# chen-bowen/instacart_next_order_recommendation

Measured on AMD Instinct MI355X. Metric: recommend_qps_top20_49k7_catalog, higher is better.
Workload: dtype f16x3 (f32 operands split into 2 f16 planes, 3 f16 MFMAs per product, f32 accumulate; fp32-level accuracy)

## Files before the change

### instacart_next_order_recommendation_amd/csrc/encoder.hip

```cpp
#include <stdlib.h>

#include <mutex>
#include <type_traits>
#include <vector>

#include "common.h"
#include "gemm_x3.h"
#include "wt_gemm.h"
#include "encoder_x3.h"

namespace icrec {

__device__ __forceinline__ int find_seq(const int32_t* __restrict__ cu, int n_seqs, int t) {
    int lo = 0, hi = n_seqs;
    while (hi - lo > 1) {
        int mid = (lo + hi) >> 1;
        if (cu[mid] <= t) lo = mid; else hi = mid;
    }
    return lo;
}

template <int H, bool SPLIT>
__device__ __forceinline__ void ln_row(float (&v)[H / 64], const float* __restrict__ g, const float* __restrict__ b,
                                       float eps, float* __restrict__ out, _Float16* __restrict__ oh,
// ... 263 lines not shown
#pragma unroll
    for (int j = 0; j < 8; ++j) {
        const _Float16 a = (_Float16)x[j];
        hi[j] = a;
        lo[j] = (_Float16)((x[j] - (float)a) * LO_SCALE);
    }
}

__device__ __forceinline__ half4 lds_read_tr(const _Float16* p) {
    typedef __fp16 fp16x4 __attribute__((__vector_size__(4 * sizeof(__fp16))));
    return __builtin_bit_cast(half4, __builtin_amdgcn_ds_read_tr16_b64_v4f16(
                                         (__attribute__((address_space(3))) fp16x4*)(reinterpret_cast<uintptr_t>(p))));
}

template <int NKT, int WAVES, bool SPLIT>
__global__ __launch_bounds__(WAVES * 64, (NKT >= 6 ? 4 : NKT == 4 ? 3 : 1)) void attention_x3_kernel(const float* __restrict__ qkv,
                                                                  const int32_t* __restrict__ cu, int heads, int H,
                                                                  float scale_log2e, float* __restrict__ ctx,
                                                                  _Float16* __restrict__ ch, _Float16* __restrict__ cl,
                                                                  const int32_t* __restrict__ order, int nlo) {
    constexpr bool RECOMP = NKT >= 6;
    __shared__ __attribute__((aligned(16))) _Float16 Kbuf[2 * NKT * 32 * 32];
    _Float16* const Kh = Kbuf;
    _Float16* const Kl = Kbuf + NKT * 32 * 32;
    __shared__ __attribute__((aligned(16))) _Float16 Vh[NKT * 32 * 32];
    __shared__ __attribute__((aligned(16))) _Float16 Vl[NKT * 32 * 32];
    __shared__ float Ls[WAVES * 32];
    constexpr bool OB = SPLIT;
    static_assert(!OB || WAVES * 2 * 32 * 32 <= 2 * NKT * 32 * 32, "the output tiles reuse the K planes");
    _Float16* const Ob = Kbuf;

    const int tid = threadIdx.x, lane = tid & 63, wave = tid >> 6;
    const int sidx = blockIdx.x / heads, hd = blockIdx.x % heads;
    const int s = order != nullptr ? order[sidx] : sidx;
    const int t0 = cu[s], L = cu[s + 1] - t0;
    const int nkt = (L + 31) >> 5;
    if (nkt > NKT || nkt <= nlo) return;
    const int qb0 = blockIdx.y * WAVES;
    if (qb0 >= nkt) return;
    const int ld = 3 * H;

    const int r = lane & 31, h = lane >> 5;
    const int qb = qb0 + wave;
    ICREC_STAMP(0, 0);
    half8 qh[2], ql[2];
    {
        int qr = qb * 32 + r;
        qr = qr < L ? qr : L - 1;
        const float* qp = qkv + (size_t)(t0 + qr) * ld + hd * DH;
#pragma unroll
        for (int ks = 0; ks < 2; ++ks) {
            const f32x4 a = *reinterpret_cast<const f32x4*>(qp + 16 * ks + 8 * h);
            const f32x4 b = *reinterpret_cast<const f32x4*>(qp + 16 * ks + 8 * h + 4);
            half4 ah, al, bh, bl;
            split_act4(a, ah, al);
            split_act4(b, bh, bl);
            qh[ks] = half8{ah[0], ah[1], ah[2], ah[3], bh[0], bh[1], bh[2], bh[3]};
            ql[ks] = half8{al[0], al[1], al[2], al[3], bl[0], bl[1], bl[2], bl[3]};
        }
    }
    ICREC_STAMP(0, 6);
    constexpr int STG = NKT * 32 * 8 / (WAVES * 64);
    static_assert(NKT * 32 * 8 % (WAVES * 64) == 0, "staging: whole rounds");
    f32x4 kreg[STG], vreg[STG];
#pragma unroll
    for (int it = 0; it < STG; ++it) {
        const int id = tid + it * WAVES * 64;
        const int key = id >> 3, c = id & 7;
        const int rr = key < L ? key : L - 1;
        const float* src = qkv + (size_t)(t0 + rr) * ld + hd * DH + c * 4;
        kreg[it] = *reinterpret_cast<const f32x4*>(src + H);
        vreg[it] = *reinterpret_cast<const f32x4*>(src + 2 * H);
    }
#ifdef ICREC_STAMPS
    asm volatile("s_waitcnt vmcnt(0)" ::: "memory");
    ICREC_STAMP(0, 7);
#endif
#pragma unroll
    for (int it = 0; it < STG; ++it) {
        const int id = tid + it * WAVES * 64;
        if (id < nkt * 32 * 8) {
            const int key = id >> 3, c = id & 7;
            half4 khi, klo, vhi, vlo;
            split_act4(kreg[it], khi, klo);
            split_act4(vreg[it], vhi, vlo);
            *reinterpret_cast<half4*>(Vh + key * 32 + c * 4) = vhi;
            *reinterpret_cast<half4*>(Vl + key * 32 + c * 4) = vlo;
            const int off = key * 32 + ((((c >> 1) ^ ((key >> 2) & 3)) << 3) | ((c & 1) << 2));
            *reinterpret_cast<half4*>(Kh + off) = khi;
            *reinterpret_cast<half4*>(Kl + off) = klo;
        }
    }
    ICREC_STAMP(0, 1);
    __syncthreads();
    ICREC_STAMP(0, 2);
    const bool active = qb < nkt;
    if (!RECOMP && !OB && !active) return;

    auto score_tile = [&](int kt, bool hi_only = false) {
        f32x16 t;
#pragma unroll
        for (int e = 0; e < 16; ++e) t[e] = 0.0f;
        const int key = kt * 32 + r;
#pragma unroll
        for (int ks = 0; ks < 2; ++ks) {
            const int off = key * 32 + (((2 * ks + h) ^ ((key >> 2) & 3)) << 3);
            const half8 kh = *reinterpret_cast<const half8*>(Kh + off);
// ... 300 lines not shown
    const long long v = strtoll(s, &end, 10);
    if (end == s) return fallback;
    return (int)(v < 0 ? 0 : v > hi ? hi : v);
}

template <bool GELU>
static void launch_linear(const float* A, int M, int K, const float* W, int N, const float* bias, float* out,
                          hipStream_t st) {
    const int mt = (M + GemmBig::BM - 1) / GemmBig::BM, nt = (N + GemmBig::BN - 1) / GemmBig::BN;
    hipLaunchKernelGGL((linear_kernel<GemmBig, GELU>), dim3(mt * nt), dim3(GemmBig::THREADS), 0, st, A, M, K, W, N,
                       bias, out, nt);
}

template <int EPI>
static void launch_wt_linear(const _Float16* Xh, const _Float16* Xl, int T, int K, const _Float16* Wp, int N,
                             const float* bias, float* out, _Float16* oh, _Float16* ol, hipStream_t st, int small_m) {
    if (T <= small_m) {
        if constexpr (EPI == 0 || EPI == 2) {
            if (N % 64 == 0 && K % 128 == 0) {
                const int nbn = N / 64;
                if (K % 256 == 0 && K >= 1024)
                    hipLaunchKernelGGL((wt_linear_half_kernel<EPI, 8>), dim3(((T + 31) / 32) * nbn), dim3(256), 0, st, Xh, Xl, T, K, Wp,
                                       N, bias, out, (const _Float16*)oh, (const _Float16*)ol, nbn);
                else if (K % 384 == 0)
                    hipLaunchKernelGGL((wt_linear_half_kernel<EPI, 6>), dim3(((T + 31) / 32) * nbn), dim3(256), 0, st, Xh, Xl, T, K, Wp,
                                       N, bias, out, (const _Float16*)oh, (const _Float16*)ol, nbn);
                else
                hipLaunchKernelGGL((wt_linear_half_kernel<EPI>), dim3(((T + 31) / 32) * nbn), dim3(256), 0, st, Xh, Xl, T, K, Wp, N,
                                   bias, out, (const _Float16*)oh, (const _Float16*)ol, nbn);
                return;
            }
        }
        const int nbn = N / 128;
        hipLaunchKernelGGL((wt_linear_kernel<1, 1, 4, EPI>), dim3(((T + 31) / 32) * nbn), dim3(256), 0, st, Xh, Xl, T, K,
                           Wp, N, bias, out, oh, ol, nbn);
    } else {
        const int nbn = N / 384;
        hipLaunchKernelGGL((wt_linear_kernel<3, 2, 1, EPI>), dim3(((T + 63) / 64) * nbn), dim3(256), 0, st, Xh, Xl, T, K,
                           Wp, N, bias, out, oh, ol, nbn);
    }
}

template <bool SPLIT, bool X3>
static void launch_attention(const float* qkv, const int32_t* cu, int n_seqs, int heads, int H, int max_seqlen,
                             float* ctx, _Float16* ch, _Float16* cl, hipStream_t st, int buckets = 31,
                             const int32_t* order = nullptr) {
    const float sl2e = (1.0f / sqrtf((float)DH)) * 1.44269504088896340736f;
    const int nkt_max = (max_seqlen + 31) / 32;
    const bool single = n_seqs == 1;
    const dim3 grid1(n_seqs * heads, 1);
#define ICREC_ATT(NKT, W, NLO)                                                                                   \
    do {                                                                                                         \
        if (X3) hipLaunchKernelGGL((attention_x3_kernel<NKT, W, SPLIT>), grid1, dim3(W * 64), 0, st, qkv, cu, heads, H, sl2e, ctx, ch, cl, order, NLO); \
        else hipLaunchKernelGGL((attention_kernel<NKT, W, SPLIT>), grid1, dim3(W * 64), 0, st, qkv, cu, heads, H, sl2e, ctx, ch, cl);      \
    } while (0)
    if ((buckets & 1) && (single ? nkt_max == 1 : true)) ICREC_ATT(1, 1, 0);
    if ((buckets & 2) && (single ? nkt_max == 2 : nkt_max >= 2)) ICREC_ATT(2, 2, 1);
    if ((buckets & 4) && (single ? (nkt_max == 3 || nkt_max == 4) : nkt_max >= 3)) ICREC_ATT(4, 4, 2);
    if (X3 && !single) {
        if ((buckets & 8) && nkt_max >= 5) ICREC_ATT(6, 6, 4);
        if ((buckets & 16) && nkt_max >= 7) ICREC_ATT(8, 8, 6);
    } else if ((buckets & 8) && nkt_max >= 5) {
        ICREC_ATT(8, 8, 4);
    }
#undef ICREC_ATT
}

}
// ... 138 lines not shown
    ICREC_REQUIRE(e && ids_dev && cu_dev && out_dev, "icrec_encode: NULL argument");
    ICREC_REQUIRE(n_seqs >= 1 && T64 >= n_seqs && T64 < (1ll << 31), "icrec_encode: bad n_seqs/total_tokens (%d, %lld)", n_seqs, (long long)T64);
    ICREC_REQUIRE(max_seqlen >= 1 && max_seqlen <= 256 && max_seqlen <= e->cfg.max_position, "icrec_encode: max_seqlen must be in [1, 256] (got %d)", max_seqlen);
    const int T = (int)T64;
    const EncWs w = enc_ws(e->cfg, T);
    if (!ws || ws_bytes < w.total) {
        set_error("icrec_encode: workspace too small (%zu < %zu)", ws_bytes, w.total);
        return ICREC_ENOMEM;
    }
    ICREC_HIP(hipSetDevice(e->device));
    hipStream_t st = (hipStream_t)stream;
    ScopedTimer whole(T_ENCODE, st);
    char* base = reinterpret_cast<char*>(ws);
    float* x = reinterpret_cast<float*>(base + w.x);
    float* qkv = reinterpret_cast<float*>(base + w.qkv);
    float* ctx = reinterpret_cast<float*>(base + w.ctx);
    float* t1 = reinterpret_cast<float*>(base + w.t1);
    float* hb = reinterpret_cast<float*>(base + w.h);
    const icrec_bert_cfg& c = e->cfg;
    const int H = c.hidden, I = c.intermediate;
    const int rows_grid = (T + 3) / 4;
    const bool x3 = c.gemm_mode == ICREC_GEMM_F16X3;
    int T_main, T_tail;
    batch_split(e, T, &T_main, &T_tail);
    const bool fuse = e->fuse, side_stream = e->side_stream;
    const int small_m = e->small_m;
    const bool qkv_res = fuse && H == 384;
    const bool lnin = fuse && H == 384 && I % 64 == 0;
    const bool split_att = x3 && side_stream && n_seqs >= 64 && max_seqlen > 128;
    Encoder::Side* sd = nullptr;
// ... 15 lines not shown
    }
    if (x3)
        hipLaunchKernelGGL((embed_ln_kernel<HID, true>), dim3(rows_grid), dim3(256), 0, st, ids_dev, cu_dev, n_seqs, T,
                           e->word, e->pos, e->type, e->eg, e->eb, c.ln_eps, c.vocab_size, c.max_position, x, xh, xl);
    else
        hipLaunchKernelGGL((embed_ln_kernel<HID, false>), dim3(rows_grid), dim3(256), 0, st, ids_dev, cu_dev, n_seqs, T,
                           e->word, e->pos, e->type, e->eg, e->eb, c.ln_eps, c.vocab_size, c.max_position, x, xh, xl);
    for (int l = 0; l < c.layers; ++l) {
        const LayerW& L = e->layers[l];
        if (x3) {
            auto qkv_stage = [&](int r0, int Tn, hipStream_t st) -> int {
                if (Tn > small_m && qkv_res) {
                    auto kern = qkv_resident_kernel;
                    if (int rc_ = ensure_dynamic_lds(reinterpret_cast<const void*>(kern), QKVR_LDS)) return rc_;
                    hipLaunchKernelGGL(kern, dim3((Tn + 63) / 64), dim3(512), QKVR_LDS, st, xh + (size_t)r0 * H,
                                       xl + (size_t)r0 * H, Tn, L.Wqkv_p, L.bqkv, qkv + (size_t)r0 * 3 * H, 3 * H);
                    return ICREC_OK;
                }
                if (lnin && l > 0 && Tn <= small_m) {
                    const LayerW& Lp = e->layers[l - 1];
                    const int nbn = 3 * H / 64;
                    hipLaunchKernelGGL((wt_linear_lnin_kernel<0, true>), dim3(((Tn + 31) / 32) * nbn), dim3(256), 0, st,
                                       (const float*)(t1 + (size_t)r0 * H), Tn, Lp.g2, Lp.b2n, c.ln_eps, xh + (size_t)r0 * H,
                                       xl + (size_t)r0 * H, L.Wqkv_p, 3 * H, L.bqkv, qkv + (size_t)r0 * 3 * H,
                                       (_Float16*)nullptr, (_Float16*)nullptr, nbn);
                    return ICREC_OK;
                }
                launch_wt_linear<0>(xh + (size_t)r0 * H, xl + (size_t)r0 * H, Tn, H, L.Wqkv_p, 3 * H, L.bqkv,
                                    qkv + (size_t)r0 * 3 * H, nullptr, nullptr, st, small_m);
                return ICREC_OK;
            };
            auto post_stage = [&](int r0, int Tn, hipStream_t st) -> int {
                float* const t1r = t1 + (size_t)r0 * H;
                _Float16 *const xhr = xh + (size_t)r0 * H, *const xlr = xl + (size_t)r0 * H;
                const _Float16 *const chr = ch + (size_t)r0 * H, *const clr = cl + (size_t)r0 * H;
                if (Tn > small_m && fuse) {
                    ScopedTimer tm(T_FFN_UP, st);
                    const int nblk = (Tn + 63) / 64;
                    auto kern = ffn_fused2_kernel<0, true>;
                    if (int rc_ = ensure_dynamic_lds(reinterpret_cast<const void*>(kern), FFN2_LDS)) return rc_;
                    const bool next_qkv = l + 1 < c.layers;
                    const LayerW& Ln = e->layers[next_qkv ? l + 1 : l];
                    hipLaunchKernelGGL(kern, dim3(nblk), dim3(512), FFN2_LDS, st, xhr, xlr, Tn, I, L.W1_p, L.b1, L.W2_p,
                                       L.b2, L.g2, L.b2n, c.ln_eps, chr, clr, L.Wo_p, L.bo, L.g1, L.b1n,
                                       next_qkv ? (const _Float16*)Ln.Wqkv_p : (const _Float16*)nullptr, (const float*)Ln.bqkv,
                                       qkv + (size_t)r0 * 3 * H, 3 * H);
                } else {
                    _Float16 *const hhr = hh + (size_t)r0 * I, *const hlr = hl + (size_t)r0 * I;
                    launch_wt_linear<2>(chr, clr, Tn, H, L.Wo_p, H, L.bo, t1r, xhr, xlr, st, small_m);
                    if (lnin && Tn <= small_m) {
                        const int nbn = I / 64;
                        hipLaunchKernelGGL((wt_linear_lnin_kernel<1, true>), dim3(((Tn + 31) / 32) * nbn), dim3(256), 0, st,
                                           (const float*)t1r, Tn, L.g1, L.b1n, c.ln_eps, xhr, xlr, L.W1_p, I, L.b1,
                                           (float*)nullptr, hhr, hlr, nbn);
                    } else {
                    hipLaunchKernelGGL(ln_wt_kernel, dim3((Tn + 15) / 16), dim3(256), 0, st, t1r, Tn, L.g1, L.b1n,
                                       c.ln_eps, xhr, xlr);
                    {
                        ScopedTimer tm(Tn > small_m ? T_FFN_UP : T_NSLOTS - 1, st);
                        launch_wt_linear<1>(xhr, xlr, Tn, H, L.W1_p, I, L.b1, nullptr, hhr, hlr, st, small_m);
                    }
// ... 14 lines not shown
                    ICREC_HIP(hipEventRecord(sd->ev_main, st));
                    ICREC_HIP(hipStreamWaitEvent(ts, sd->ev_main, 0));
                }
                if (l == 0 || !tail_qkv_in_fused)
                    if (int rc_ = qkv_stage(T_main, T_tail, ts)) return rc_;
                ICREC_HIP(hipEventRecord(sd->ev_qkv_tail, ts));
            } else if (T_tail && (l == 0 || !tail_qkv_in_fused)) {
                if (int rc_ = qkv_stage(T_main, T_tail, st)) return rc_;
            }
            if (l == 0 || !qkv_in_fused)
                if (int rc_ = qkv_stage(0, T_main, st)) return rc_;
            if (T_tail && use_side) ICREC_HIP(hipStreamWaitEvent(st, sd->ev_qkv_tail, 0));
            if (split_att && use_side) {
                ICREC_HIP(hipEventRecord(sd->ev_q, st));
                ICREC_HIP(hipStreamWaitEvent(sd->side, sd->ev_q, 0));
                launch_attention<true, true>(qkv, cu_dev, n_seqs, c.heads, H, max_seqlen, ctx, ch, cl, sd->side, 7 | 16, order);
                ICREC_HIP(hipEventRecord(sd->ev_sa, sd->side));
                launch_attention<true, true>(qkv, cu_dev, n_seqs, c.heads, H, max_seqlen, ctx, ch, cl, st, 8, order);
                ICREC_HIP(hipStreamWaitEvent(st, sd->ev_sa, 0));
            } else {
                launch_attention<true, true>(qkv, cu_dev, n_seqs, c.heads, H, max_seqlen, ctx, ch, cl, st, 31, order);
            }
            if (T_tail) {
                if (use_side) {
                    ICREC_HIP(hipEventRecord(sd->ev_att, st));
                    ICREC_HIP(hipStreamWaitEvent(ts, sd->ev_att, 0));
                }
                if (int rc_ = post_stage(T_main, T_tail, ts)) return rc_;
            }
            if (int rc_ = post_stage(0, T_main, st)) return rc_;
            if (T_tail && use_side && l + 1 == c.layers) {
                ICREC_HIP(hipEventRecord(sd->ev_tail, ts));
                ICREC_HIP(hipStreamWaitEvent(st, sd->ev_tail, 0));
            }
        } else {
            launch_linear<false>(x, T, H, L.Wqkv, 3 * H, L.bqkv, qkv, st);
            launch_attention<false, false>(qkv, cu_dev, n_seqs, c.heads, H, max_seqlen, ctx, ch, cl, st);
            launch_linear<false>(ctx, T, H, L.Wo, H, L.bo, t1, st);
            hipLaunchKernelGGL((add_ln_kernel<HID, false>), dim3(rows_grid), dim3(256), 0, st, t1, x, T, L.g1, L.b1n,
                               c.ln_eps, xh, xl);
            {
                ScopedTimer tm(T_FFN_UP, st);
                launch_linear<true>(x, T, H, L.W1, I, L.b1, hb, st);
            }
            launch_linear<false>(hb, T, I, L.W2, H, L.b2, t1, st);
            hipLaunchKernelGGL((add_ln_kernel<HID, false>), dim3(rows_grid), dim3(256), 0, st, t1, x, T, L.g2, L.b2n,
                               c.ln_eps, xh, xl);
        }
    }
    if (x3) hipLaunchKernelGGL((pool_norm_kernel<HID, true>), dim3(n_seqs), dim3(HID), 0, st, x, xh, xl, cu_dev, c.n_normalize, out_dev);
    else hipLaunchKernelGGL((pool_norm_kernel<HID, false>), dim3(n_seqs), dim3(HID), 0, st, x, xh, xl, cu_dev, c.n_normalize, out_dev);
    ICREC_HIP(hipGetLastError());
// ... 5 lines not shown
```

### instacart_next_order_recommendation_amd/csrc/encoder_x3.h

```cpp
#pragma once
#include <type_traits>

#include "wt_gemm.h"

namespace icrec {

__device__ __forceinline__ float gelu16_wt(float x) {
    const float t = fminf(fabsf(x), 5.75f);
    float q = -1.428101063e-08f;
    q = fmaf(q, t, 4.683960178e-07f);
    q = fmaf(q, t, -6.560040814e-06f);
    q = fmaf(q, t, 4.923233760e-05f);
    q = fmaf(q, t, -1.793856253e-04f);
    q = fmaf(q, t, -2.251562182e-04f);
    q = fmaf(q, t, 7.249582803e-03f);
    q = fmaf(q, t, -5.267105742e-02f);
    q = fmaf(q, t, -4.591336602e-01f);
    q = fmaf(q, t, -1.151116827e+00f);
    q = fmaf(q, t, 2.960897358e-07f);
    const float e = __builtin_amdgcn_exp2f(q);
    return fmaf(fabsf(x) * -8.0f, e, fmaxf(x * 16.0f, 0.0f));
}
__device__ __forceinline__ void gelu_split4(const f32x4& acc, const f32x4& bias, half4& hi, half4& lo) {
    f32x4 s;
// ... 282 lines not shown
            if (ok) {
                *reinterpret_cast<half4*>(xh + tok * 384 + feat) = hi;
                *reinterpret_cast<half4*>(xl + tok * 384 + feat) = lo;
            }
        }
}

constexpr int LN_LD = 388;

template <int NTW, int TTW, int D, int EPI>
__global__ __launch_bounds__(256, 2) void wt_linear_kernel(const _Float16* __restrict__ Xh,
                                                           const _Float16* __restrict__ Xl, int T, int K,
                                                           const _Float16* __restrict__ Wp, int N,
                                                           const float* __restrict__ bias, float* __restrict__ out,
                                                           _Float16* __restrict__ oh, _Float16* __restrict__ ol,
                                                           int n_blocks_n) {
    constexpr bool STAGED = (NTW == 3 && TTW == 2 && EPI != 1);
    constexpr int SM = (STAGED && 32 * LN_LD * 4 > XRing<TTW>::BYTES) ? 32 * LN_LD * 4 : XRing<TTW>::BYTES;
    __shared__ __attribute__((aligned(16))) char smem[SM];
    const int lane = threadIdx.x & 63, q = wave_uniform(threadIdx.x >> 6), c = lane & 15, g = lane >> 4;
    const int bid = xcd_remap(blockIdx.x, gridDim.x);
    const int mt = bid / n_blocks_n, nb = bid % n_blocks_n;
    const int64_t m0 = (int64_t)mt * (32 * TTW);
    const int nt0 = (nb * 4 + q) * NTW;
    Acc32 acc[NTW][TTW];
    wt_kloop<NTW, TTW, D>(acc, Wp, nt0, K, Xh, Xl, m0, T, smem);
    if constexpr (EPI == 2) {
        if constexpr (NTW == 3 && TTW == 2) {
            ResRows r0, r1;
            wt_res_rows_load(r0, q, 0, oh + nb * 384, ol + nb * 384, m0, T);
            wt_res_rows_load(r1, q, 1, oh + nb * 384, ol + nb * 384, m0, T);
// ... 19 lines not shown
                    if (EPI == 0) b = *reinterpret_cast<const f32x4*>(bias + n0 + fl);
#pragma unroll
                    for (int ti = 0; ti < 2; ++ti) {
                        f32x4 v;
#pragma unroll
                        for (int j = 0; j < 4; ++j)
                            v[j] = EPI == 2 ? acc[i][tt].t[fi][ti][j] * WT_UNSCALE : fmaf(acc[i][tt].t[fi][ti][j], WT_UNSCALE, b[j]);
                        *reinterpret_cast<f32x4*>(stage + (ti * 16 + c) * LN_LD + fl) = v;
                    }
                }
            __syncthreads();
#pragma unroll
            for (int k = 0; k < 12; ++k) {
                const int f = threadIdx.x + 256 * k, row = f / 96, ch = f - row * 96;
                const int64_t tok = m0 + tt * 32 + row;
                if (tok < T)
                    *reinterpret_cast<f32x4*>(out + tok * N + n0 + ch * 4) = *reinterpret_cast<const f32x4*>(stage + row * LN_LD + ch * 4);
            }
            if (tt == 0) __syncthreads();
        }
        ICREC_STAMP(0, 30);
        return;
    }

#pragma unroll
    for (int i = 0; i < NTW; ++i)
#pragma unroll
        for (int fi = 0; fi < 2; ++fi) {
            const int feat = (nt0 + i) * 32 + fi * 16 + 4 * g;
            f32x4 b = f32x4{0.0f, 0.0f, 0.0f, 0.0f};
            if (EPI != 2) b = *reinterpret_cast<const f32x4*>(bias + feat);
#pragma unroll
            for (int tt = 0; tt < TTW; ++tt)
#pragma unroll
                for (int ti = 0; ti < 2; ++ti) {
                    const int64_t tok = m0 + tt * 32 + ti * 16 + c;
                    if (tok < T) {
                        if (EPI == 1) {
                            half4 hi, lo;
                            gelu_split4(acc[i][tt].t[fi][ti], b, hi, lo);
                            *reinterpret_cast<half4*>(oh + tok * N + feat) = hi;
                            *reinterpret_cast<half4*>(ol + tok * N + feat) = lo;
                        } else {
                            f32x4 v;
#pragma unroll
                            for (int j = 0; j < 4; ++j)
                                v[j] = EPI == 2 ? acc[i][tt].t[fi][ti][j] * WT_UNSCALE : fmaf(acc[i][tt].t[fi][ti][j], WT_UNSCALE, b[j]);
                            *reinterpret_cast<f32x4*>(out + tok * N + feat) = v;
                        }
                    }
                }
        }
    ICREC_STAMP(0, 30);
}

constexpr int FFN2_X_BYTES = 2 * FFN2_XPLANE;

template <int NT>
__device__ __forceinline__ void ffn_x_stage(char* Xs, const _Float16* __restrict__ xh, const _Float16* __restrict__ xl,
                                            int64_t m0, int64_t T) {
    constexpr int N = 64 * 48 / NT;
    u32x4 vh[N], vl[N];
#pragma unroll
// ... 22 lines not shown
__device__ __forceinline__ void ffn_x_frag(XFrag& x, const char* Xs, const int (&xb)[2][2], int tt, int ks) {
#pragma unroll
    for (int ti = 0; ti < 2; ++ti) {
        const int pos = (xb[tt][ti] ^ ((ks & 3) << 6)) + (ks >> 2) * 256;
        x.h[ti] = *reinterpret_cast<const half8*>(Xs + pos);
        x.l[ti] = *reinterpret_cast<const half8*>(Xs + FFN2_XPLANE + pos);
    }
}

template <int EPI, int D = 4>
__global__ __launch_bounds__(256, 2) void wt_linear_half_kernel(const _Float16* __restrict__ Xh,
                                                                    const _Float16* __restrict__ Xl, int T, int K,
                                                                    const _Float16* __restrict__ Wp, int N,
                                                                    const float* __restrict__ bias, float* __restrict__ out,
                                                                    const _Float16* __restrict__ rh,
                                                                    const _Float16* __restrict__ rl, int n_blocks_n) {
    __shared__ __attribute__((aligned(16))) char smem[XRing<1>::BYTES];
    const int lane = threadIdx.x & 63, q = wave_uniform(threadIdx.x >> 6), c = lane & 15, g = lane >> 4;
    const int bid = xcd_remap(blockIdx.x, gridDim.x);
    const int mt = bid / n_blocks_n, nb = bid % n_blocks_n;
    const int64_t m0 = (int64_t)mt * 32;
    const int ft = nb * 4 + q, nt = ft >> 1, fi = ft & 1;
    const unsigned lo8 = lane * 8;
    const int KS = K / 32, nslab = K / 64;
    const _Float16* const wp = Wp + wt_frag_off(nt, 0, KS) + (size_t)fi * (2 * WT_FRAG);
    static_assert(D == 4 || D == 6 || D == 8, "ring depth: 4, 6 (K a multiple of 384) or 8 (K a multiple of 256) k-steps");
    half8 wh[D], wl[D];
    auto w_load1 = [&](int slot, int ks) {
        const _Float16* p = wp + (size_t)ks * (4 * WT_FRAG);
        wh[slot] = *reinterpret_cast<const half8*>(p + lo8);
        wl[slot] = *reinterpret_cast<const half8*>(p + WT_FRAG + lo8);
// ... 59 lines not shown
    const f32x4 b = *reinterpret_cast<const f32x4*>(bias + feat);
#pragma unroll
    for (int ti = 0; ti < 2; ++ti) {
        const int64_t tok = m0 + ti * 16 + c;
        if (tok < T) {
            f32x4 v;
            if constexpr (EPI == 2) {
                const half4 a = *reinterpret_cast<const half4*>(rh + tok * N + feat);
                const half4 d = *reinterpret_cast<const half4*>(rl + tok * N + feat);
#pragma unroll
                for (int j = 0; j < 4; ++j) v[j] = (acc[ti][j] + res_init_val(a[j], d[j], b[j])) * WT_UNSCALE;
            } else {
#pragma unroll
                for (int j = 0; j < 4; ++j) v[j] = fmaf(acc[ti][j], WT_UNSCALE, b[j]);
            }
            *reinterpret_cast<f32x4*>(out + tok * N + feat) = v;
        }
    }
}

constexpr int LNIN_XPLANE = 32 * 768;
template <int EPI, bool HALF = false>
__global__ __launch_bounds__(256, 2) void wt_linear_lnin_kernel(const float* __restrict__ a, int T,
                                                                const float* __restrict__ gam,
                                                                const float* __restrict__ bet, float eps,
                                                                _Float16* __restrict__ xh, _Float16* __restrict__ xl,
                                                                const _Float16* __restrict__ Wp, int N,
                                                                const float* __restrict__ bias, float* __restrict__ out,
                                                                _Float16* __restrict__ oh, _Float16* __restrict__ ol,
                                                                int n_blocks_n) {
    constexpr int KS1 = 12;
    __shared__ __attribute__((aligned(16))) char Xs[2 * LNIN_XPLANE];
    const int tid = threadIdx.x, lane = tid & 63, wq = wave_uniform(tid >> 6), c = lane & 15, g = lane >> 4;
    const int bid = xcd_remap(blockIdx.x, gridDim.x);
    const int mt = bid / n_blocks_n, nb = bid % n_blocks_n;
    const int64_t m0 = (int64_t)mt * 32;
    const int ft = nb * 4 + wq;
    const int nt = HALF ? ft >> 1 : ft, hf = ft & 1;
    const unsigned lo8 = lane * 8;
    constexpr int RD = 8;
    WFrag w[RD][1];
    const _Float16* const wp1[1] = {Wp + wt_frag_off(nt, 0, KS1)};
    auto w_ring_load = [&](int slot, int ks) {
        if constexpr (HALF) {
            const _Float16* p = wp1[0] + (size_t)ks * (4 * WT_FRAG) + (size_t)hf * (2 * WT_FRAG);
// ... 109 lines not shown
    for (int fi = 0; fi < (HALF ? 1 : 2); ++fi) {
        const int feat = nt * 32 + (HALF ? hf : fi) * 16 + 4 * g;
#pragma unroll
        for (int ti = 0; ti < 2; ++ti) {
            const int64_t tok = m0 + ti * 16 + c;
            if (tok < T) {
                if (EPI == 1) {
                    half4 hi, lo;
                    gelu_split4(S.t[fi][ti], bv[fi], hi, lo);
                    *reinterpret_cast<half4*>(oh + tok * N + feat) = hi;
                    *reinterpret_cast<half4*>(ol + tok * N + feat) = lo;
                } else {
                    f32x4 v;
#pragma unroll
                    for (int j = 0; j < 4; ++j) v[j] = fmaf(S.t[fi][ti][j], WT_UNSCALE, bv[fi][j]);
                    *reinterpret_cast<f32x4*>(out + tok * N + feat) = v;
                }
            }
        }
    }
}

constexpr int QKVR_STG_LD = 36;
constexpr int QKVR_STG_BYTES = 32 * QKVR_STG_LD * 4;
constexpr int QKVR_LDS = FFN2_X_BYTES + 8 * QKVR_STG_BYTES;

__device__ __forceinline__ void qkv_block_walk(const char* Xs, float* stg, const _Float16* __restrict__ Wp,
                                               const float* __restrict__ bias, float* __restrict__ out, int N, int64_t m0,
                                               int64_t T, int wave, int lane, int c, int g, unsigned lo8) {
    constexpr int KS1 = 12;
    const int NT = N / 32;
    int xb[2][2];
    ffn_x_bases(xb, c, g);
    WFrag w[4][1];
    {
        const _Float16* const wp0[1] = {Wp + wt_frag_off(wave, 0, KS1)};
#pragma unroll
        for (int d = 0; d < 4; ++d) w_load<1>(w[d], wp0, d, lo8);
    }
    for (int nt = wave; nt < NT; nt += 8) {
        const int nn = nt + 8 < NT ? nt + 8 : nt;
        const _Float16* const wp1[1] = {Wp + wt_frag_off(nt, 0, KS1)};
        const _Float16* const wpn[1] = {Wp + wt_frag_off(nn, 0, KS1)};
        f32x4 bv[2];
// ... 31 lines not shown
                    for (int j = 0; j < 4; ++j) v[j] = fmaf(S[0][tt].t[fi][ti][j], WT_UNSCALE, bv[fi][j]);
                    *reinterpret_cast<f32x4*>(stg + (ti * 16 + c) * QKVR_STG_LD + fi * 16 + 4 * g) = v;
                }
            lds_order();
            f32x4 o[4];
#pragma unroll
            for (int k = 0; k < 4; ++k) {
                const int f = lane + 64 * k;
                o[k] = *reinterpret_cast<const f32x4*>(stg + (f >> 3) * QKVR_STG_LD + (f & 7) * 4);
            }
            lds_order();
#pragma unroll
            for (int k = 0; k < 4; ++k) {
                const int f = lane + 64 * k;
                const int64_t tok = m0 + tt * 32 + (f >> 3);
                if (tok < T) *reinterpret_cast<f32x4*>(out + tok * N + nt * 32 + (f & 7) * 4) = o[k];
            }
        }
    }
}

constexpr int FFN_IC = 128;
constexpr int FFN2_HPLANE = 64 * 256;
constexpr int FFN2_HBUF = 2 * FFN2_HPLANE;
constexpr int FFN2_LDS = FFN2_X_BYTES + 2 * FFN2_HBUF;
static_assert(FFN2_LDS == 160 * 1024, "fused FFN LDS budget");

__device__ __forceinline__ void bar_lds() {
    asm volatile("s_waitcnt lgkmcnt(0)\n\ts_barrier" ::: "memory");
}

// ... 2 lines not shown
                                                            int T, int I,
                                                            const _Float16* __restrict__ W1p,
                                                            const float* __restrict__ b1,
                                                            const _Float16* __restrict__ W2p,
                                                            const float* __restrict__ b2,
                                                            const float* __restrict__ gam,
                                                            const float* __restrict__ bet, float eps,
                                                            const _Float16* __restrict__ ch = nullptr,
                                                            const _Float16* __restrict__ cl = nullptr,
                                                            const _Float16* __restrict__ Wop = nullptr,
                                                            const float* __restrict__ bo = nullptr,
                                                            const float* __restrict__ gam1 = nullptr,
                                                            const float* __restrict__ bet1 = nullptr,
                                                            const _Float16* __restrict__ Wqp = nullptr,
                                                            const float* __restrict__ bq = nullptr,
                                                            float* __restrict__ qkv_out = nullptr, int Nq = 0) {
    constexpr int KS1 = 12;
    extern __shared__ __attribute__((aligned(16))) char smem2[];
    char* const Xs = smem2;
    char* const Hs = smem2 + FFN2_X_BYTES;
    const int tid = threadIdx.x, lane = tid & 63, wave = wave_uniform(tid >> 6), q = wave & 3;
    int c = lane & 15, g = lane >> 4;
    const bool producer = wave < 4;
    const int64_t m0 = (int64_t)blockIdx.x * 64;
    const int NC = I / FFN_IC, KS2 = I / 32;

    ICREC_STAMP(0, 0);
    ICREC_STAMP(4, 0);
    ICREC_STAMP_RT(0, 62);
    if constexpr ((VAR & 64) != 0) {
        __builtin_amdgcn_s_sleep(127);
// ... 282 lines not shown
#pragma unroll
        for (int i = 0; i < 3; ++i)
#pragma unroll
            for (int fi = 0; fi < 2; ++fi)
#pragma unroll
                for (int ti = 0; ti < 2; ++ti)
                    *reinterpret_cast<f32x4*>(Xs + ((q * 12) + (i * 2 + fi) * 2 + ti) * 1024 + lane * 16) = Y[i][1].t[fi][ti];
        __syncthreads();
        wt_ln_block<8, 2, 0>(Y, q, 0, wave, xh, xl, m0, T, gam, bet, eps, Hs, [] { __syncthreads(); }, tid, Wqp != nullptr ? Xs : nullptr);
    }
    ICREC_STAMP(0, 30);
    ICREC_STAMP(4, 30);
    if (Wqp != nullptr) {
        __syncthreads();
        asm volatile("" : "+v"(c), "+v"(g), "+v"(lo8));
        qkv_block_walk(Xs, reinterpret_cast<float*>(Hs + wave * QKVR_STG_BYTES), Wqp, bq, qkv_out, Nq, m0, T, wave, lane, c, g, lo8);
    }
    ICREC_STAMP(0, 43);
    ICREC_STAMP(4, 43);
    ICREC_STAMP_RT(0, 63);
}

__global__ __launch_bounds__(512, 2) void qkv_resident_kernel(const _Float16* __restrict__ xh,
                                                              const _Float16* __restrict__ xl, int T,
                                                              const _Float16* __restrict__ Wp,
                                                              const float* __restrict__ bias,
                                                              float* __restrict__ out, int N) {
    extern __shared__ __attribute__((aligned(16))) char smem2[];
    char* const Xs = smem2;
    const int tid = threadIdx.x, lane = tid & 63, wave = wave_uniform(tid >> 6), c = lane & 15, g = lane >> 4;
    float* const stg = reinterpret_cast<float*>(smem2 + FFN2_X_BYTES + wave * QKVR_STG_BYTES);
    const int64_t m0 = (int64_t)blockIdx.x * 64;
    ffn_x_stage<512>(Xs, xh, xl, m0, T);
    __syncthreads();
    qkv_block_walk(Xs, stg, Wp, bias, out, N, m0, T, wave, lane, c, g, lane * 8);
}

__global__ __launch_bounds__(256) void pack_weights_kernel(const float* __restrict__ w, int N, int K,
                                                           _Float16* __restrict__ out) {
    const int KS = K / 32;
    const size_t n = (size_t)(N / 16) * KS * 64;
    for (size_t id = (size_t)blockIdx.x * 256 + threadIdx.x; id < n; id += (size_t)gridDim.x * 256) {
        const size_t fr = id >> 6;
        const int lane = (int)(id & 63), c = lane & 15, g = lane >> 4;
        const int nt16 = (int)(fr / KS), ks = (int)(fr % KS);
        const float* src = w + (size_t)(nt16 * 16 + c) * K + ks * 32 + 8 * g;
        half8 hi, lo;
#pragma unroll
        for (int j = 0; j < 8; ++j) {
            _Float16 a, b;
// ... 12 lines not shown
```

Baseline: 110,600.

## Store QKV as pre-split f16 head planes and load attention tiles directly into LDS

The QKV producer epilogues now split each f32 output into hi/lo f16 values and write them into per-head, token-major planes instead of a row-major f32 buffer. The attention kernel then reads Q directly as half8 and streams K/V planes into LDS with global_load_lds, with the swizzle applied at the source address. This removes the per-call f32 load, split and LDS store staging in attention and halves the bytes it reads. The cost is extra split work and scattered stores in the GEMM epilogues. The non-x3 fallback path still passes the f32 qkv buffer, and the K/V LDS buffers are merged into one array.

Result: no change. 110,200, median of 6 (-0.4%).

```diff
diff --git a/instacart_next_order_recommendation_amd/csrc/encoder.hip b/instacart_next_order_recommendation_amd/csrc/encoder.hip
--- a/instacart_next_order_recommendation_amd/csrc/encoder.hip
+++ b/instacart_next_order_recommendation_amd/csrc/encoder.hip
@@ -301,17 +301,18 @@
 }
 
 template <int NKT, int WAVES, bool SPLIT>
-__global__ __launch_bounds__(WAVES * 64, (NKT >= 6 ? 4 : NKT == 4 ? 3 : 1)) void attention_x3_kernel(const float* __restrict__ qkv,
+__global__ __launch_bounds__(WAVES * 64, (NKT >= 6 ? 4 : NKT == 4 ? 3 : 1)) void attention_x3_kernel(const _Float16* __restrict__ qkv,
+                                                                  int64_t pt,
                                                                   const int32_t* __restrict__ cu, int heads, int H,
                                                                   float scale_log2e, float* __restrict__ ctx,
                                                                   _Float16* __restrict__ ch, _Float16* __restrict__ cl,
                                                                   const int32_t* __restrict__ order, int nlo) {
     constexpr bool RECOMP = NKT >= 6;
-    __shared__ __attribute__((aligned(16))) _Float16 Kbuf[2 * NKT * 32 * 32];
+    __shared__ __attribute__((aligned(16))) _Float16 Kbuf[4 * NKT * 32 * 32];
     _Float16* const Kh = Kbuf;
     _Float16* const Kl = Kbuf + NKT * 32 * 32;
-    __shared__ __attribute__((aligned(16))) _Float16 Vh[NKT * 32 * 32];
-    __shared__ __attribute__((aligned(16))) _Float16 Vl[NKT * 32 * 32];
+    _Float16* const Vh = Kbuf + 2 * NKT * 32 * 32;
+    _Float16* const Vl = Kbuf + 3 * NKT * 32 * 32;
     __shared__ float Ls[WAVES * 32];
     constexpr bool OB = SPLIT;
     static_assert(!OB || WAVES * 2 * 32 * 32 <= 2 * NKT * 32 * 32, "the output tiles reuse the K planes");
@@ -325,59 +326,39 @@
     if (nkt > NKT || nkt <= nlo) return;
     const int qb0 = blockIdx.y * WAVES;
     if (qb0 >= nkt) return;
-    const int ld = 3 * H;
+    const int64_t lo_off = (int64_t)3 * H * pt;
 
     const int r = lane & 31, h = lane >> 5;
     const int qb = qb0 + wave;
     ICREC_STAMP(0, 0);
+    {
+        const int nb = (nkt * 32 + 15) >> 4;
+#pragma unroll
+        for (int it = 0; it < 8 * NKT / WAVES; ++it) {
+            const int p = wave + it * WAVES, pl = p / (2 * NKT), rb = p - pl * (2 * NKT);
+            if (rb < nb) {
+                const int key = rb * 16 + (lane >> 2), rr = key < L ? key : L - 1;
+                const int ch = (lane & 3) ^ (pl < 2 ? (key >> 2) & 3 : 0);
+                const _Float16* src = qkv + ((int64_t)((pl < 2 ? 1 : 2) * heads + hd) * pt + t0 + rr) * 32 + ch * 8 +
+                                      ((pl & 1) ? lo_off : 0);
+                __builtin_amdgcn_global_load_lds((const __attribute__((address_space(1))) void*)src,
+                                                 (__attribute__((address_space(3))) void*)(Kbuf + (size_t)p * 512), 16, 0, 0);
+            }
+        }
+    }
     half8 qh[2], ql[2];
     {
         int qr = qb * 32 + r;
         qr = qr < L ? qr : L - 1;
-        const float* qp = qkv + (size_t)(t0 + qr) * ld + hd * DH;
+        const _Float16* qp = qkv + ((int64_t)hd * pt + t0 + qr) * 32;
 #pragma unroll
         for (int ks = 0; ks < 2; ++ks) {
-            const f32x4 a = *reinterpret_cast<const f32x4*>(qp + 16 * ks + 8 * h);
-            const f32x4 b = *reinterpret_cast<const f32x4*>(qp + 16 * ks + 8 * h + 4);
-            half4 ah, al, bh, bl;
-            split_act4(a, ah, al);
-            split_act4(b, bh, bl);
-            qh[ks] = half8{ah[0], ah[1], ah[2], ah[3], bh[0], bh[1], bh[2], bh[3]};
-            ql[ks] = half8{al[0], al[1], al[2], al[3], bl[0], bl[1], bl[2], bl[3]};
-        }
-    }
-    ICREC_STAMP(0, 6);
-    constexpr int STG = NKT * 32 * 8 / (WAVES * 64);
-    static_assert(NKT * 32 * 8 % (WAVES * 64) == 0, "staging: whole rounds");
-    f32x4 kreg[STG], vreg[STG];
-#pragma unroll
-    for (int it = 0; it < STG; ++it) {
-        const int id = tid + it * WAVES * 64;
-        const int key = id >> 3, c = id & 7;
-        const int rr = key < L ? key : L - 1;
-        const float* src = qkv + (size_t)(t0 + rr) * ld + hd * DH + c * 4;
-        kreg[it] = *reinterpret_cast<const f32x4*>(src + H);
-        vreg[it] = *reinterpret_cast<const f32x4*>(src + 2 * H);
-    }
-#ifdef ICREC_STAMPS
+            qh[ks] = *reinterpret_cast<const half8*>(qp + 16 * ks + 8 * h);
+            ql[ks] = *reinterpret_cast<const half8*>(qp + lo_off + 16 * ks + 8 * h);
+        }
+    }
+    static_assert(8 * NKT % WAVES == 0, "K / V pieces: whole rounds");
     asm volatile("s_waitcnt vmcnt(0)" ::: "memory");
-    ICREC_STAMP(0, 7);
-#endif
-#pragma unroll
-    for (int it = 0; it < STG; ++it) {
-        const int id = tid + it * WAVES * 64;
-        if (id < nkt * 32 * 8) {
-            const int key = id >> 3, c = id & 7;
-            half4 khi, klo, vhi, vlo;
-            split_act4(kreg[it], khi, klo);
-            split_act4(vreg[it], vhi, vlo);
-            *reinterpret_cast<half4*>(Vh + key * 32 + c * 4) = vhi;
-            *reinterpret_cast<half4*>(Vl + key * 32 + c * 4) = vlo;
-            const int off = key * 32 + ((((c >> 1) ^ ((key >> 2) & 3)) << 3) | ((c & 1) << 2));
-            *reinterpret_cast<half4*>(Kh + off) = khi;
-            *reinterpret_cast<half4*>(Kl + off) = klo;
-        }
-    }
     ICREC_STAMP(0, 1);
     __syncthreads();
     ICREC_STAMP(0, 2);
@@ -708,35 +689,36 @@
 
 template <int EPI>
 static void launch_wt_linear(const _Float16* Xh, const _Float16* Xl, int T, int K, const _Float16* Wp, int N,
-                             const float* bias, float* out, _Float16* oh, _Float16* ol, hipStream_t st, int small_m) {
+                             const float* bias, float* out, _Float16* oh, _Float16* ol, hipStream_t st, int small_m,
+                             int64_t pt = 0) {
     if (T <= small_m) {
         if constexpr (EPI == 0 || EPI == 2) {
             if (N % 64 == 0 && K % 128 == 0) {
                 const int nbn = N / 64;
                 if (K % 256 == 0 && K >= 1024)
                     hipLaunchKernelGGL((wt_linear_half_kernel<EPI, 8>), dim3(((T + 31) / 32) * nbn), dim3(256), 0, st, Xh, Xl, T, K, Wp,
-                                       N, bias, out, (const _Float16*)oh, (const _Float16*)ol, nbn);
+                                       N, bias, out, (const _Float16*)oh, (const _Float16*)ol, nbn, oh, pt);
                 else if (K % 384 == 0)
                     hipLaunchKernelGGL((wt_linear_half_kernel<EPI, 6>), dim3(((T + 31) / 32) * nbn), dim3(256), 0, st, Xh, Xl, T, K, Wp,
-                                       N, bias, out, (const _Float16*)oh, (const _Float16*)ol, nbn);
+                                       N, bias, out, (const _Float16*)oh, (const _Float16*)ol, nbn, oh, pt);
                 else
                 hipLaunchKernelGGL((wt_linear_half_kernel<EPI>), dim3(((T + 31) / 32) * nbn), dim3(256), 0, st, Xh, Xl, T, K, Wp, N,
-                                   bias, out, (const _Float16*)oh, (const _Float16*)ol, nbn);
+                                   bias, out, (const _Float16*)oh, (const _Float16*)ol, nbn, oh, pt);
                 return;
             }
         }
         const int nbn = N / 128;
         hipLaunchKernelGGL((wt_linear_kernel<1, 1, 4, EPI>), dim3(((T + 31) / 32) * nbn), dim3(256), 0, st, Xh, Xl, T, K,
-                           Wp, N, bias, out, oh, ol, nbn);
+                           Wp, N, bias, out, oh, ol, nbn, pt);
     } else {
         const int nbn = N / 384;
         hipLaunchKernelGGL((wt_linear_kernel<3, 2, 1, EPI>), dim3(((T + 63) / 64) * nbn), dim3(256), 0, st, Xh, Xl, T, K,
-                           Wp, N, bias, out, oh, ol, nbn);
+                           Wp, N, bias, out, oh, ol, nbn, pt);
     }
 }
 
 template <bool SPLIT, bool X3>
-static void launch_attention(const float* qkv, const int32_t* cu, int n_seqs, int heads, int H, int max_seqlen,
+static void launch_attention(const float* qkv, int64_t T, const int32_t* cu, int n_seqs, int heads, int H, int max_seqlen,
                              float* ctx, _Float16* ch, _Float16* cl, hipStream_t st, int buckets = 31,
                              const int32_t* order = nullptr) {
     const float sl2e = (1.0f / sqrtf((float)DH)) * 1.44269504088896340736f;
@@ -745,7 +727,7 @@
     const dim3 grid1(n_seqs * heads, 1);
 #define ICREC_ATT(NKT, W, NLO)                                                                                   \
     do {                                                                                                         \
-        if (X3) hipLaunchKernelGGL((attention_x3_kernel<NKT, W, SPLIT>), grid1, dim3(W * 64), 0, st, qkv, cu, heads, H, sl2e, ctx, ch, cl, order, NLO); \
+        if (X3) hipLaunchKernelGGL((attention_x3_kernel<NKT, W, SPLIT>), grid1, dim3(W * 64), 0, st, (const _Float16*)qkv, T, cu, heads, H, sl2e, ctx, ch, cl, order, NLO); \
         else hipLaunchKernelGGL((attention_kernel<NKT, W, SPLIT>), grid1, dim3(W * 64), 0, st, qkv, cu, heads, H, sl2e, ctx, ch, cl);      \
     } while (0)
     if ((buckets & 1) && (single ? nkt_max == 1 : true)) ICREC_ATT(1, 1, 0);
@@ -914,6 +896,7 @@
     char* base = reinterpret_cast<char*>(ws);
     float* x = reinterpret_cast<float*>(base + w.x);
     float* qkv = reinterpret_cast<float*>(base + w.qkv);
+    _Float16* const qkvp = reinterpret_cast<_Float16*>(qkv);
     float* ctx = reinterpret_cast<float*>(base + w.ctx);
     float* t1 = reinterpret_cast<float*>(base + w.t1);
     float* hb = reinterpret_cast<float*>(base + w.h);
@@ -959,7 +942,7 @@
                     auto kern = qkv_resident_kernel;
                     if (int rc_ = ensure_dynamic_lds(reinterpret_cast<const void*>(kern), QKVR_LDS)) return rc_;
                     hipLaunchKernelGGL(kern, dim3((Tn + 63) / 64), dim3(512), QKVR_LDS, st, xh + (size_t)r0 * H,
-                                       xl + (size_t)r0 * H, Tn, L.Wqkv_p, L.bqkv, qkv + (size_t)r0 * 3 * H, 3 * H);
+                                       xl + (size_t)r0 * H, Tn, L.Wqkv_p, L.bqkv, qkvp + (size_t)r0 * 32, 3 * H, (int64_t)T);
                     return ICREC_OK;
                 }
                 if (lnin && l > 0 && Tn <= small_m) {
@@ -967,12 +950,12 @@
                     const int nbn = 3 * H / 64;
                     hipLaunchKernelGGL((wt_linear_lnin_kernel<0, true>), dim3(((Tn + 31) / 32) * nbn), dim3(256), 0, st,
                                        (const float*)(t1 + (size_t)r0 * H), Tn, Lp.g2, Lp.b2n, c.ln_eps, xh + (size_t)r0 * H,
-                                       xl + (size_t)r0 * H, L.Wqkv_p, 3 * H, L.bqkv, qkv + (size_t)r0 * 3 * H,
-                                       (_Float16*)nullptr, (_Float16*)nullptr, nbn);
+                                       xl + (size_t)r0 * H, L.Wqkv_p, 3 * H, L.bqkv, (float*)nullptr,
+                                       qkvp + (size_t)r0 * 32, (_Float16*)nullptr, nbn, (int64_t)T);
                     return ICREC_OK;
                 }
-                launch_wt_linear<0>(xh + (size_t)r0 * H, xl + (size_t)r0 * H, Tn, H, L.Wqkv_p, 3 * H, L.bqkv,
-                                    qkv + (size_t)r0 * 3 * H, nullptr, nullptr, st, small_m);
+                launch_wt_linear<0>(xh + (size_t)r0 * H, xl + (size_t)r0 * H, Tn, H, L.Wqkv_p, 3 * H, L.bqkv, nullptr,
+                                    qkvp + (size_t)r0 * 32, nullptr, st, small_m, (int64_t)T);
                 return ICREC_OK;
             };
             auto post_stage = [&](int r0, int Tn, hipStream_t st) -> int {
@@ -989,7 +972,7 @@
                     hipLaunchKernelGGL(kern, dim3(nblk), dim3(512), FFN2_LDS, st, xhr, xlr, Tn, I, L.W1_p, L.b1, L.W2_p,
                                        L.b2, L.g2, L.b2n, c.ln_eps, chr, clr, L.Wo_p, L.bo, L.g1, L.b1n,
                                        next_qkv ? (const _Float16*)Ln.Wqkv_p : (const _Float16*)nullptr, (const float*)Ln.bqkv,
-                                       qkv + (size_t)r0 * 3 * H, 3 * H);
+                                       qkvp + (size_t)r0 * 32, 3 * H, (int64_t)T);
                 } else {
                     _Float16 *const hhr = hh + (size_t)r0 * I, *const hlr = hl + (size_t)r0 * I;
                     launch_wt_linear<2>(chr, clr, Tn, H, L.Wo_p, H, L.bo, t1r, xhr, xlr, st, small_m);
@@ -1034,12 +1017,12 @@
             if (split_att && use_side) {
                 ICREC_HIP(hipEventRecord(sd->ev_q, st));
                 ICREC_HIP(hipStreamWaitEvent(sd->side, sd->ev_q, 0));
-                launch_attention<true, true>(qkv, cu_dev, n_seqs, c.heads, H, max_seqlen, ctx, ch, cl, sd->side, 7 | 16, order);
+                launch_attention<true, true>(qkv, T, cu_dev, n_seqs, c.heads, H, max_seqlen, ctx, ch, cl, sd->side, 7 | 16, order);
                 ICREC_HIP(hipEventRecord(sd->ev_sa, sd->side));
-                launch_attention<true, true>(qkv, cu_dev, n_seqs, c.heads, H, max_seqlen, ctx, ch, cl, st, 8, order);
+                launch_attention<true, true>(qkv, T, cu_dev, n_seqs, c.heads, H, max_seqlen, ctx, ch, cl, st, 8, order);
                 ICREC_HIP(hipStreamWaitEvent(st, sd->ev_sa, 0));
             } else {
-                launch_attention<true, true>(qkv, cu_dev, n_seqs, c.heads, H, max_seqlen, ctx, ch, cl, st, 31, order);
+                launch_attention<true, true>(qkv, T, cu_dev, n_seqs, c.heads, H, max_seqlen, ctx, ch, cl, st, 31, order);
             }
             if (T_tail) {
                 if (use_side) {
@@ -1055,7 +1038,7 @@
             }
         } else {
             launch_linear<false>(x, T, H, L.Wqkv, 3 * H, L.bqkv, qkv, st);
-            launch_attention<false, false>(qkv, cu_dev, n_seqs, c.heads, H, max_seqlen, ctx, ch, cl, st);
+            launch_attention<false, false>(qkv, T, cu_dev, n_seqs, c.heads, H, max_seqlen, ctx, ch, cl, st);
             launch_linear<false>(ctx, T, H, L.Wo, H, L.bo, t1, st);
             hipLaunchKernelGGL((add_ln_kernel<HID, false>), dim3(rows_grid), dim3(256), 0, st, t1, x, T, L.g1, L.b1n,
                                c.ln_eps, xh, xl);
diff --git a/instacart_next_order_recommendation_amd/csrc/encoder_x3.h b/instacart_next_order_recommendation_amd/csrc/encoder_x3.h
--- a/instacart_next_order_recommendation_amd/csrc/encoder_x3.h
+++ b/instacart_next_order_recommendation_amd/csrc/encoder_x3.h
@@ -4,6 +4,15 @@
 #include "wt_gemm.h"
 
 namespace icrec {
+
+__device__ __forceinline__ void qkv_plane_store(_Float16* __restrict__ q, int N, int64_t pt, int64_t tok, int feat,
+                                                const f32x4& v) {
+    half4 hi, lo;
+    split_act4(v, hi, lo);
+    _Float16* const p = q + ((int64_t)(feat >> 5) * pt + tok) * 32 + (feat & 31);
+    *reinterpret_cast<half4*>(p) = hi;
+    *reinterpret_cast<half4*>(p + (int64_t)N * pt) = lo;
+}
 
 __device__ __forceinline__ float gelu16_wt(float x) {
     const float t = fminf(fabsf(x), 5.75f);
@@ -320,7 +329,7 @@
                                                            const _Float16* __restrict__ Wp, int N,
                                                            const float* __restrict__ bias, float* __restrict__ out,
                                                            _Float16* __restrict__ oh, _Float16* __restrict__ ol,
-                                                           int n_blocks_n) {
+                                                           int n_blocks_n, int64_t pt = 0) {
     constexpr bool STAGED = (NTW == 3 && TTW == 2 && EPI != 1);
     constexpr int SM = (STAGED && 32 * LN_LD * 4 > XRing<TTW>::BYTES) ? 32 * LN_LD * 4 : XRing<TTW>::BYTES;
     __shared__ __attribute__((aligned(16))) char smem[SM];
@@ -370,8 +379,11 @@
             for (int k = 0; k < 12; ++k) {
                 const int f = threadIdx.x + 256 * k, row = f / 96, ch = f - row * 96;
                 const int64_t tok = m0 + tt * 32 + row;
-                if (tok < T)
-                    *reinterpret_cast<f32x4*>(out + tok * N + n0 + ch * 4) = *reinterpret_cast<const f32x4*>(stage + row * LN_LD + ch * 4);
+                if (tok < T) {
+                    const f32x4 v = *reinterpret_cast<const f32x4*>(stage + row * LN_LD + ch * 4);
+                    if (EPI == 0) qkv_plane_store(oh, N, pt, tok, n0 + ch * 4, v);
+                    else *reinterpret_cast<f32x4*>(out + tok * N + n0 + ch * 4) = v;
+                }
             }
             if (tt == 0) __syncthreads();
         }
@@ -402,7 +414,8 @@
 #pragma unroll
                             for (int j = 0; j < 4; ++j)
                                 v[j] = EPI == 2 ? acc[i][tt].t[fi][ti][j] * WT_UNSCALE : fmaf(acc[i][tt].t[fi][ti][j], WT_UNSCALE, b[j]);
-                            *reinterpret_cast<f32x4*>(out + tok * N + feat) = v;
+                            if (EPI == 0) qkv_plane_store(oh, N, pt, tok, feat, v);
+                            else *reinterpret_cast<f32x4*>(out + tok * N + feat) = v;
                         }
                     }
                 }
@@ -455,7 +468,8 @@
                                                                     const _Float16* __restrict__ Wp, int N,
                                                                     const float* __restrict__ bias, float* __restrict__ out,
                                                                     const _Float16* __restrict__ rh,
-                                                                    const _Float16* __restrict__ rl, int n_blocks_n) {
+                                                                    const _Float16* __restrict__ rl, int n_blocks_n,
+                                                                    _Float16* __restrict__ qp = nullptr, int64_t pt = 0) {
     __shared__ __attribute__((aligned(16))) char smem[XRing<1>::BYTES];
     const int lane = threadIdx.x & 63, q = wave_uniform(threadIdx.x >> 6), c = lane & 15, g = lane >> 4;
     const int bid = xcd_remap(blockIdx.x, gridDim.x);
@@ -545,7 +559,8 @@
 #pragma unroll
                 for (int j = 0; j < 4; ++j) v[j] = fmaf(acc[ti][j], WT_UNSCALE, b[j]);
             }
-            *reinterpret_cast<f32x4*>(out + tok * N + feat) = v;
+            if constexpr (EPI == 0) qkv_plane_store(qp, N, pt, tok, feat, v);
+            else *reinterpret_cast<f32x4*>(out + tok * N + feat) = v;
         }
     }
 }
@@ -559,7 +574,7 @@
                                                                 const _Float16* __restrict__ Wp, int N,
                                                                 const float* __restrict__ bias, float* __restrict__ out,
                                                                 _Float16* __restrict__ oh, _Float16* __restrict__ ol,
-                                                                int n_blocks_n) {
+                                                                int n_blocks_n, int64_t pt = 0) {
     constexpr int KS1 = 12;
     __shared__ __attribute__((aligned(16))) char Xs[2 * LNIN_XPLANE];
     const int tid = threadIdx.x, lane = tid & 63, wq = wave_uniform(tid >> 6), c = lane & 15, g = lane >> 4;
@@ -699,7 +714,8 @@
                     f32x4 v;
 #pragma unroll
                     for (int j = 0; j < 4; ++j) v[j] = fmaf(S.t[fi][ti][j], WT_UNSCALE, bv[fi][j]);
-                    *reinterpret_cast<f32x4*>(out + tok * N + feat) = v;
+                    if (EPI == 0) qkv_plane_store(oh, N, pt, tok, feat, v);
+                    else *reinterpret_cast<f32x4*>(out + tok * N + feat) = v;
                 }
             }
         }
@@ -711,8 +727,9 @@
 constexpr int QKVR_LDS = FFN2_X_BYTES + 8 * QKVR_STG_BYTES;
 
 __device__ __forceinline__ void qkv_block_walk(const char* Xs, float* stg, const _Float16* __restrict__ Wp,
-                                               const float* __restrict__ bias, float* __restrict__ out, int N, int64_t m0,
-                                               int64_t T, int wave, int lane, int c, int g, unsigned lo8) {
+                                               const float* __restrict__ bias, _Float16* __restrict__ out, int N,
+                                               int64_t pt, int64_t m0, int64_t T, int wave, int lane, int c, int g,
+                                               unsigned lo8) {
     constexpr int KS1 = 12;
     const int NT = N / 32;
     int xb[2][2];
@@ -774,7 +791,7 @@
             for (int k = 0; k < 4; ++k) {
                 const int f = lane + 64 * k;
                 const int64_t tok = m0 + tt * 32 + (f >> 3);
-                if (tok < T) *reinterpret_cast<f32x4*>(out + tok * N + nt * 32 + (f & 7) * 4) = o[k];
+                if (tok < T) qkv_plane_store(out, N, pt, tok, nt * 32 + (f & 7) * 4, o[k]);
             }
         }
     }
@@ -807,7 +824,8 @@
                                                             const float* __restrict__ bet1 = nullptr,
                                                             const _Float16* __restrict__ Wqp = nullptr,
                                                             const float* __restrict__ bq = nullptr,
-                                                            float* __restrict__ qkv_out = nullptr, int Nq = 0) {
+                                                            _Float16* __restrict__ qkv_out = nullptr, int Nq = 0,
+                                                            int64_t qkv_pt = 0) {
     constexpr int KS1 = 12;
     extern __shared__ __attribute__((aligned(16))) char smem2[];
     char* const Xs = smem2;
@@ -1120,7 +1138,8 @@
     if (Wqp != nullptr) {
         __syncthreads();
         asm volatile("" : "+v"(c), "+v"(g), "+v"(lo8));
-        qkv_block_walk(Xs, reinterpret_cast<float*>(Hs + wave * QKVR_STG_BYTES), Wqp, bq, qkv_out, Nq, m0, T, wave, lane, c, g, lo8);
+        qkv_block_walk(Xs, reinterpret_cast<float*>(Hs + wave * QKVR_STG_BYTES), Wqp, bq, qkv_out, Nq, qkv_pt, m0, T, wave, lane, c, g,
+                       lo8);
     }
     ICREC_STAMP(0, 43);
     ICREC_STAMP(4, 43);
@@ -1131,7 +1150,7 @@
                                                               const _Float16* __restrict__ xl, int T,
                                                               const _Float16* __restrict__ Wp,
                                                               const float* __restrict__ bias,
-                                                              float* __restrict__ out, int N) {
+                                                              _Float16* __restrict__ out, int N, int64_t pt) {
     extern __shared__ __attribute__((aligned(16))) char smem2[];
     char* const Xs = smem2;
     const int tid = threadIdx.x, lane = tid & 63, wave = wave_uniform(tid >> 6), c = lane & 15, g = lane >> 4;
@@ -1139,7 +1158,7 @@
     const int64_t m0 = (int64_t)blockIdx.x * 64;
     ffn_x_stage<512>(Xs, xh, xl, m0, T);
     __syncthreads();
-    qkv_block_walk(Xs, stg, Wp, bias, out, N, m0, T, wave, lane, c, g, lane * 8);
+    qkv_block_walk(Xs, stg, Wp, bias, out, N, pt, m0, T, wave, lane, c, g, lane * 8);
 }
 
 __global__ __launch_bounds__(256) void pack_weights_kernel(const float* __restrict__ w, int N, int K,
```
